# yg838457845/ORB_SLAM2-Chinese-annotation

Measured on AMD Instinct MI355X. Metric: frames/sec (extract+match) at 1241×376, 1000 feat/frame; 1/2/4/8 GPU, higher is better.
Workload: dtype u8; 1 GPU; C4: 1241x376 KITTI-shaped synthetic stream, 1000 feat/frame, SearchByProjection vs 5000-point local map per frame; distinct_frames_per_gpu=8192, frames_per_launch=1024, parallelism=single rank; no collective (one process, one GPU)

## Files before the change

orb_slam2-chinese-annotation_amd/csrc/extractor_kernels.hip:

```cpp
#include <stdlib.h>
#include <type_traits>
#include <algorithm>
#include "orb_device.h"
#include "orb_plan.h"
#include "orb_kernels.h"
#include "orb_pattern_data.h"
#include "../../include/orb_abi.h"

#define PYR_TW 128
#ifndef PYR_IMAGES_PER_WG
#define PYR_IMAGES_PER_WG 16
#endif
#define PYR_TH 32
#ifndef PYR_TARGET_WGS
#define PYR_TARGET_WGS 0
#endif
#define PYR_SROWS 44
#define PYR_SW 44
#define PYR_SROWS_WIDE 64
#define PYR_SW_WIDE 64

__global__ __launch_bounds__(256) void k_pyr_resize_generic(
    const uint8_t* __restrict__ src, long long srcImgPitch, int srcStride, int sw, int sh,
    uint8_t* __restrict__ dst, long long dstImgPitch, int dstStride, int dw, int dh,
// ... 1042 lines not shown
#if !FC_ROWMAJOR
      if (fresh)
        sc64[valid ? (o >> 3) : trashS] = last ? outsideLast : 0ull;
#endif
#if FC_ROWMAJOR
      const uint32_t X = __builtin_amdgcn_perm(rp[1], rp[0], 0x07050301u);
      const uint32_t Y = __builtin_amdgcn_perm(rp[3], rp[2], 0x07050301u);
      const uint32_t fails = ((X >> 7) & 0x01010101u) | ((Y >> 3) & 0x10101010u);
      uint32_t mk = ~((fails * 0x01020408u) >> 24) &
                    (valid ? (last ? (1u << nvLast) - 1u : 0xFFu) : 0u);
      const int cnt = __builtin_popcount(mk);
      int incl = wave_incl_scan(cnt);
      __asm__ volatile("" : "+v"(incl));
      int pos = nq + incl - cnt;
      while (mk) {
        const int j = __builtin_ctz(mk);
        mk &= mk - 1u;
        queue[pos++] = (uint16_t)(off + j);
      }
      nq += __builtin_amdgcn_readlane(incl, 63);
#else
      const unsigned long long vm = __ballot(valid), vIn = __ballot(valid && !last);
#pragma unroll
      for (int j = 0; j < 8; ++j) {
        const uint32_t w = rp[j >> 1];
        const bool sgn = (j & 1) ? ((int)w >= 0) : ((short)(w & 0xFFFFu) >= 0);
        const unsigned long long bj = __ballot(sgn) & (j < nvLast ? vm : vIn);
        const int pos = (int)__builtin_amdgcn_mbcnt_hi((uint32_t)(bj >> 32),
                                                       __builtin_amdgcn_mbcnt_lo((uint32_t)bj, (uint32_t)nq));
        queue[lane_select(bj, pos, trashQ)] = (uint16_t)(off + j);
        nq += __popcll(bj);
      }
#endif
      }
      k += kInc;
      off += dOff;
      if (k >= nK) {
        k -= nK;
        off += wrapOff;
      }
      if (nq > FC_QCAP - 512 || g0 + 64 >= nG) {
        wave_lds_sync();
        flush(t, fresh);
        wave_lds_sync();
      }
    }
  };
  auto nms = [&](int t) {
    for (int i = lane; i < 2 * ih; i += 64) bits[i] = 0;
    wave_lds_sync();
    const bool dense = nc > FC_CCAP;
    const int nItems = dense ? ih * iw : nc;
    for (int j = lane; j < nItems; j += 64) {
      int x, y, off;
      if (dense) {
        y = (int)(((float)j + 0.5f) * invW);
        x = j - y * iw;
        off = (y + 3) * P + (x + 8);
      } else {
        off = corners[j];
        const int ry = (int)(((float)off + 0.5f) * invP);
        y = ry - 3;
        x = off - ry * P - 8;
      }
      const uint8_t* cp = sc + off;
      const int m = cp[0];
      const int r0 = cp[-P - 1], r1 = cp[-P], r2 = cp[-P + 1], r3 = cp[-1], r4 = cp[1],
                r5 = cp[P - 1], r6 = cp[P], r7 = cp[P + 1];
      if (m <= t || m < 2) continue;
      const bool L = x > 0, Rt = x < iw - 1, U = y > 0, D = y < ih - 1;
      const int nb[8] = {(U && L) ? r0 : 0, U ? r1 : 0, (U && Rt) ? r2 : 0, L ? r3 : 0,
                         Rt ? r4 : 0, (D && L) ? r5 : 0, D ? r6 : 0, (D && Rt) ? r7 : 0};
      bool ok = true;
#pragma unroll
      for (int k = 0; k < 8; ++k) ok = ok && !(nb[k] > t && nb[k] >= m);
      if (ok) atomicOr(&bits[2 * y + (x >> 5)], 1u << (x & 31));
    }
    wave_lds_sync();
  };
  uint32_t* out = cellKeys + slot * plan.keyCap;
  auto nms_emit = [&](int t) -> int {
    const bool dense = nc > FC_CCAP;
    const int nItems = dense ? ih * iw : nc;
    const uint32_t kx0 = (uint32_t)(cd.x0 + 3), ky0 = (uint32_t)(cd.y0 + 3);
    int nOut = 0;
    for (int j0 = 0; j0 < nItems; j0 += 64) {
      const int j = j0 + lane;
      bool ok = false;
      int x = 0, y = 0, m = 0;
      if (j < nItems) {
        int off;
        if (dense) {
          y = (int)(((float)j + 0.5f) * invW);
          x = j - y * iw;
          off = (y + 3) * P + (x + 8);
        } else {
          off = corners[j];
          const int ry = (int)(((float)off + 0.5f) * invP);
          y = ry - 3;
          x = off - ry * P - 8;
        }
        int oq = off - P - 1;
        if (PT) __asm__ volatile("" : "+v"(oq));
        const uint8_t* cq = sc + oq;
        m = cq[P + 1];
        const int nb[8] = {cq[0], cq[1], cq[2], cq[P], cq[P + 2], cq[2 * P], cq[2 * P + 1],
                           cq[2 * P + 2]};
        ok = m > t && m >= 2;
#pragma unroll
        for (int k = 0; k < 8; ++k) ok = ok && !(nb[k] > t && nb[k] >= m);
      }
      const unsigned long long bal = __ballot(ok);
      const int pos = nOut + (int)__builtin_amdgcn_mbcnt_hi((uint32_t)(bal >> 32),
                                                            __builtin_amdgcn_mbcnt_lo((uint32_t)bal, 0u));
      if (ok) out[pos] = pack_key(kx0 + x, ky0 + y, m - 1);
      nOut += __popcll(bal);
    }
    return nOut;
  };
  auto compact = [&]() -> int {
    unsigned long long row = 0ull;
    if (lane < ih) {
      const uint2 w = *reinterpret_cast<const uint2*>(bits + 2 * lane);
      row = (unsigned long long)w.x | ((unsigned long long)w.y << 32);
    }
    const int cnt = __popcll(row);
    const int incl = wave_incl_scan(cnt);
    const int total = __builtin_amdgcn_readlane(incl, 63);
    int o = incl - cnt;
    const uint8_t* srow = sc + (lane + 3) * P + 8;
    const uint32_t kx = (uint32_t)(cd.x0 + 3), ky = (uint32_t)(cd.y0 + 3 + lane);
    while (row) {
      const int x0 = __builtin_ctzll(row);
      row &= row - 1;
      const bool two = row != 0;
      const int x1 = two ? __builtin_ctzll(row) : x0;
      if (two) row &= row - 1;
      const int m0 = srow[x0], m1 = srow[x1];
      out[o] = pack_key(kx + x0, ky, m0 - 1);
      if (two) out[o + 1] = pack_key(kx + x1, ky, m1 - 1);
      o += two ? 2 : 1;
    }
    return total;
  };
#if FC_ROWMAJOR
  (void)nms;
  (void)compact;
#endif
  fast_pass(ti, true);
#if FC_ROWMAJOR
  int n = nms_emit(ti);
#else
  nms(ti);
  int n = compact();
#endif
  if (n == 0 && tm != ti) {
    nc = 0;
    fast_pass(tm, false);
#if FC_ROWMAJOR
    n = nms_emit(tm);
#else
    nms(tm);
    n = compact();
#endif
  }
  if (lane == 0) cellCount[slot] = n;
  ci = ciNext;
  wave_lds_sync();
  }
}

struct OctNode {
  int16_t x0, y0, x1, y1;
  int cnt;
  int seq;
};

__device__ __forceinline__ int oct_quad(uint32_t key, const OctNode& n) {
  const int kx = key_x(key) - 16, ky = key_y(key) - 16;
  const int mx = n.x0 + ((n.x1 - n.x0 + 1) >> 1);
  const int my = n.y0 + ((n.y1 - n.y0 + 1) >> 1);
  return (kx < mx ? 0 : 1) + (ky < my ? 0 : 2);
}

__device__ __forceinline__ OctNode oct_child(const OctNode& p, int q, int cnt, int seq) {
  const int mx = p.x0 + ((p.x1 - p.x0 + 1) >> 1);
  const int my = p.y0 + ((p.y1 - p.y0 + 1) >> 1);
  OctNode c;
  c.x0 = (int16_t)((q & 1) ? mx : p.x0);
  c.x1 = (int16_t)((q & 1) ? p.x1 : mx);
  c.y0 = (int16_t)((q & 2) ? my : p.y0);
  c.y1 = (int16_t)((q & 2) ? p.y1 : my);
  c.cnt = cnt;
  c.seq = seq;
  return c;
}

__device__ int block_scan_array(int* a, int n, int* tmp) {
  const int T = blockDim.x, t = threadIdx.x;
  const int per = (n + T - 1) / T;
  const int b = min(t * per, n), e = min(b + per, n);
  int s = 0;
  for (int i = b; i < e; ++i) s += a[i];
  int total;
  int ex = block_excl_scan(s, tmp, &total);
  for (int i = b; i < e; ++i) {
    const int v = a[i];
    a[i] = ex;
    ex += v;
  }
  __syncthreads();
  return total;
}

__device__ void block_scan2(int* a, int na, int* b, int nb, int extra, int* tmp, int* totA,
                            int* totB, int* totX) {
  const int T = blockDim.x, t = threadIdx.x;
  const int pa = (na + T - 1) / T, pb = (nb + T - 1) / T;
  const int ba = min(t * pa, na), ea = min(ba + pa, na);
  const int bb = min(t * pb, nb), eb = min(bb + pb, nb);
  __syncthreads();
  int sa = 0, sb = 0;
  for (int i = ba; i < ea; ++i) sa += a[i];
  for (int i = bb; i < eb; ++i) sb += b[i];
  const int l = lane_id(), w = t >> 6, nw = (T + 63) >> 6;
  const int ia = wave_incl_scan(sa), ib = wave_incl_scan(sb), ix = wave_incl_scan(extra);
  if (l == 63) {
    tmp[w] = ia;
    tmp[16 + w] = ib;
    tmp[32 + w] = ix;
  }
  __syncthreads();
  if (t < 3) {
    int acc = 0;
    for (int i = 0; i < nw; ++i) {
      const int v = tmp[16 * t + i];
      tmp[16 * t + i] = acc;
      acc += v;
    }
    tmp[48 + t] = acc;
  }
  __syncthreads();
  int xa = tmp[w] + ia - sa, xb = tmp[16 + w] + ib - sb;
  *totA = tmp[48];
  *totB = tmp[49];
  *totX = tmp[50];
  for (int i = ba; i < ea; ++i) {
    const int v = a[i];
    a[i] = xa;
    xa += v;
  }
  for (int i = bb; i < eb; ++i) {
    const int v = b[i];
    b[i] = xb;
    xb += v;
  }
  __syncthreads();
}

__device__ void block_bitonic_desc(unsigned long long* v, int n2) {
  for (int k = 2; k <= n2; k <<= 1) {
    for (int j = k >> 1; j > 0; j >>= 1) {
      for (int i = threadIdx.x; i < n2; i += blockDim.x) {
        const int ixj = i ^ j;
        if (ixj > i) {
          const unsigned long long a = v[i], b = v[ixj];
          const bool descBlock = (i & k) == 0;
          if (descBlock ? (a < b) : (a > b)) {
            v[i] = b;
            v[ixj] = a;
          }
        }
      }
      __syncthreads();
    }
  }
}

#define OCT_RANK_MAX 512
template <int RQ>
__device__ __forceinline__ void oct_rank_by_count(unsigned long long* sortBuf, int ncand, int t, int T) {
  unsigned long long mine[RQ];
  int rank[RQ];
#pragma unroll
  for (int q = 0; q < RQ; ++q) {
    const int j = t + q * T;
    mine[q] = j < ncand ? sortBuf[j] : 0ull;
    rank[q] = 0;
  }
  for (int i = 0; i < ncand; ++i) {
    const unsigned long long k = sortBuf[i];
#pragma unroll
    for (int q = 0; q < RQ; ++q) rank[q] += k > mine[q];
  }
  __syncthreads();
#pragma unroll
  for (int q = 0; q < RQ; ++q)
    if (t + q * T < ncand) sortBuf[rank[q]] = mine[q];
  __syncthreads();
}

#define OCT_MAX_PASSES 512
#define OCT_REG_KEYS 8
#ifndef OCT_BATCH_THREADS
#define OCT_BATCH_THREADS 256
#endif
#ifndef OCT_REG_THREADS
#define OCT_REG_THREADS 512
#endif

template <bool REG, bool GNODES>
__global__ __launch_bounds__(512) void k_octree(
    OrbPlanDesc plan, const int32_t* __restrict__ cellCount, const uint32_t* __restrict__ cellKeys,
    uint32_t* __restrict__ gKeys, uint16_t* __restrict__ gNid, int ldsKeyCap, int nodeCapMax,
    int maxCellsPerLevel, uint32_t* __restrict__ outKeys, int32_t* __restrict__ outCount,
    int32_t* __restrict__ errFlag, int levelBeg, int maxPasses, unsigned char* __restrict__ gNodes,
    long long nodeStride) {
  extern __shared__ __attribute__((aligned(16))) unsigned char smem[];
  __shared__ int tmp[52];
  __shared__ int sh[8];
  const int l = levelBeg + blockIdx.y, img = blockIdx.x, T = blockDim.x, t = threadIdx.x;
  const OrbLevelDesc& L = plan.lv[l];
  const int NC = nodeCapMax;
  int n2 = 1;
  while (n2 < NC) n2 <<= 1;
  unsigned char* p = GNODES ? gNodes + ((long long)img * plan.nlevels + l) * nodeStride : smem;
  unsigned long long* sortBuf = (unsigned long long*)p; p += (size_t)n2 * 8;
  OctNode* A = (OctNode*)p; p += (size_t)NC * sizeof(OctNode);
  OctNode* B = (OctNode*)p; p += (size_t)NC * sizeof(OctNode);
  int* q4 = (int*)p; p += (size_t)NC * 16;
  int* g0 = (int*)p; p += (size_t)NC * 4;
  int* g1 = (int*)p; p += (size_t)NC * 4;
  int* g2 = (int*)p; p += (size_t)NC * 4;
  int* rk = (int*)p; p += (size_t)NC * 4;
  int* cellBase = (int*)p; p += (size_t)((maxCellsPerLevel + 3) & ~3) * 4;
  if (GNODES) p = smem;
  uint32_t* Klds = (uint32_t*)p; p += (size_t)ldsKeyCap * 4;
  uint16_t* Nlds = (uint16_t*)p;

  const int cb = L.cellBeg, nc = L.cellEnd - L.cellBeg;
  const long long cellSlot0 = (long long)img * plan.ncells + cb;
  for (int i = t; i < nc; i += T) cellBase[i] = cellCount[cellSlot0 + i];
  __syncthreads();
  const int n = block_scan_array(cellBase, nc, tmp);
  uint32_t* K;
  uint16_t* NID;
  if (n <= ldsKeyCap) {
    K = Klds;
    NID = Nlds;
  } else {
    K = gKeys + cellSlot0 * plan.keyCap;
    NID = gNid + cellSlot0 * plan.keyCap;
  }
  errFlag += img;
  for (int c = t; c < nc; c += T) {
    const int cnt = cellCount[cellSlot0 + c], base = cellBase[c];
    const uint32_t* src = cellKeys + (cellSlot0 + c) * plan.keyCap;
    for (int i = 0; i < cnt; ++i) K[base + i] = src[i];
  }
  const bool inReg = REG && n <= OCT_REG_KEYS * T;
  uint32_t kr[OCT_REG_KEYS];
  int nr[OCT_REG_KEYS];
  auto each_key = [&](auto&& f) {
    if (inReg) {
#pragma unroll
      for (int i = 0; i < OCT_REG_KEYS; ++i) {
        const int k = t + i * T;
        if (k < n) f(kr[i], nr[i], k);
      }
    } else {
      for (int k = t; k < n; k += T) {
        const uint32_t key = K[k];
        int nid = NID[k];
        f(key, nid, k);
        NID[k] = (uint16_t)nid;
      }
    }
  };
  __syncthreads();
  if (inReg) {
#pragma unroll
    for (int i = 0; i < OCT_REG_KEYS; ++i) {
      const int k = t + i * T;
      kr[i] = k < n ? K[k] : 0u;
      nr[i] = 0;
    }
  }
  const int nIni = L.nIni;
  const float hX = L.hX;
  for (int i = t; i < nIni; i += T) g0[i] = 0;
  __syncthreads();
  each_key([&](uint32_t key, int& nid, int) {
    const float xr = (float)(key_x(key) - 16);
    const int r = min((int)__fdiv_rn(xr, hX), nIni - 1);
    nid = r;
    atomicAdd(&g0[r], 1);
  });
  __syncthreads();
  if (t == 0) {
    int a = 0;
    for (int i = 0; i < nIni; ++i) {
      g1[i] = a;
      if (g0[i] > 0) {
        OctNode nd;
        nd.x0 = (int16_t)(int)(hX * (float)i);
        nd.x1 = (int16_t)(int)(hX * (float)(i + 1));
        nd.y0 = 0;
        nd.y1 = (int16_t)L.Hr;
        nd.cnt = g0[i];
        nd.seq = i;
        A[a++] = nd;
      }
    }
    sh[0] = a;
  }
  __syncthreads();
  each_key([&](uint32_t, int& nid, int) { nid = g1[nid]; });
  int alive = sh[0];
  const int N = L.quota;
  int seqNext = nIni;
  bool finalPhase = false;
  int pass = 0;
  __syncthreads();
  for (; pass < maxPasses; ++pass) {
    const int prev = alive;
    if (!finalPhase) {
      for (int i = t; i < alive * 4; i += T) q4[i] = 0;
      __syncthreads();
      each_key([&](uint32_t key, int& nid, int) {
        const OctNode nd = A[nid];
        if (nd.cnt > 1) atomicAdd(&q4[nid * 4 + oct_quad(key, nd)], 1);
      });
      __syncthreads();
      int nteLocal = 0;
      for (int a = t; a < alive; a += T) {
        int nce = 0;
        if (A[a].cnt > 1) {
#pragma unroll
          for (int q = 0; q < 4; ++q) {
            const int c = q4[a * 4 + q];
            nce += c > 0;
            nteLocal += c > 1;
          }
        }
        g0[a] = nce;
        g1[a] = A[a].cnt > 1 ? 0 : 1;
      }
      int nToExpand, S, NM;
      block_scan2(g0, alive, g1, alive, nteLocal, tmp, &S, &NM, &nToExpand);
      if (S + NM > NC) {
        if (t == 0) atomicOr(errFlag, 2);
        break;
      }
      for (int a = t; a < alive; a += T) {
        const OctNode nd = A[a];
        if (nd.cnt > 1) {
          int pos = g0[a];
#pragma unroll
          for (int q = 0; q < 4; ++q) {
            const int c = q4[a * 4 + q];
            if (c > 0) {
              const int ni = S - 1 - pos;
              B[ni] = oct_child(nd, q, c, seqNext + pos);
              q4[a * 4 + q] = ni;
              ++pos;
            }
          }
        } else {
          const int ni = S + g1[a];
          B[ni] = nd;
          q4[a * 4] = ni;
        }
      }
      __syncthreads();
      each_key([&](uint32_t key, int& nid, int) {
        const OctNode nd = A[nid];
        nid = q4[nid * 4 + (nd.cnt > 1 ? oct_quad(key, nd) : 0)];
      });
      __syncthreads();
      OctNode* sw = A; A = B; B = sw;
      alive = S + NM;
      seqNext += S;
      if (alive >= N || alive == prev) break;
      if (alive + nToExpand * 3 > N) finalPhase = true;
    } else {
      if (seqNext >= (1 << 24)) {
        if (t == 0) atomicOr(errFlag, 8);
        break;
      }
      for (int a = t; a < alive; a += T) g0[a] = A[a].cnt > 1 ? 1 : 0;
      __syncthreads();
      const int ncand = block_scan_array(g0, alive, tmp);
      if (ncand == 0) break;
      int m2 = 1;
      while (m2 < ncand) m2 <<= 1;
      for (int i = t; i < m2; i += T) sortBuf[i] = 0ull;
      __syncthreads();
      for (int a = t; a < alive; a += T) {
        const OctNode nd = A[a];
        if (nd.cnt > 1)
          sortBuf[g0[a]] = ((unsigned long long)nd.cnt << 40) |
                           ((unsigned long long)(uint32_t)nd.seq << 16) | (unsigned)a;
        q4[a * 4 + 0] = q4[a * 4 + 1] = q4[a * 4 + 2] = q4[a * 4 + 3] = 0;
        rk[a] = 0x7fffffff;
      }
      __syncthreads();
      if (ncand <= OCT_RANK_MAX) {
        if (T >= OCT_RANK_MAX)
          oct_rank_by_count<1>(sortBuf, ncand, t, T);
        else if (T >= 256)
          oct_rank_by_count<OCT_RANK_MAX / 256>(sortBuf, ncand, t, T);
        else
          oct_rank_by_count<OCT_RANK_MAX / 128>(sortBuf, ncand, t, T);
      } else {
        block_bitonic_desc(sortBuf, m2);
      }
      for (int j = t; j < ncand; j += T) rk[(int)(sortBuf[j] & 0xFFFF)] = j;
      each_key([&](uint32_t key, int& nid, int) {
        const OctNode nd = A[nid];
        if (nd.cnt > 1) atomicAdd(&q4[nid * 4 + oct_quad(key, nd)], 1);
      });
      if (t == 0) sh[1] = ncand - 1;
      __syncthreads();
      for (int j = t; j < ncand; j += T) {
        const int a = (int)(sortBuf[j] & 0xFFFF);
        int nce = 0;
#pragma unroll
        for (int q = 0; q < 4; ++q) nce += q4[a * 4 + q] > 0;
        g1[j] = nce;
        g2[j] = nce - 1;
      }
      __syncthreads();
      block_scan_array(g2, ncand, tmp);
      for (int j = t; j < ncand; j += T)
        if (alive + g2[j] + (g1[j] - 1) >= N) atomicMin(&sh[1], j);
      __syncthreads();
      const int jstop = sh[1];
      for (int j = t; j < ncand; j += T)
        if (j > jstop) g1[j] = 0;
      for (int a = t; a < alive; a += T) g2[a] = (rk[a] <= jstop) ? 0 : 1;
      int S, keep, unused;
      block_scan2(g1, ncand, g2, alive, 0, tmp, &S, &keep, &unused);
      if (S + keep > NC) {
        if (t == 0) atomicOr(errFlag, 2);
        break;
      }
      for (int a = t; a < alive; a += T) {
        const OctNode nd = A[a];
        const int j = rk[a];
        if (j <= jstop) {
          int pos = g1[j];
#pragma unroll
          for (int q = 0; q < 4; ++q) {
            const int c = q4[a * 4 + q];
            if (c > 0) {
              const int ni = S - 1 - pos;
              B[ni] = oct_child(nd, q, c, seqNext + pos);
              q4[a * 4 + q] = ni;
              ++pos;
            }
          }
        } else {
          const int ni = S + g2[a];
          B[ni] = nd;
          q4[a * 4] = ni;
        }
      }
      __syncthreads();
      each_key([&](uint32_t key, int& nid, int) {
        const OctNode nd = A[nid];
        nid = q4[nid * 4 + (rk[nid] <= jstop ? oct_quad(key, nd) : 0)];
      });
      __syncthreads();
      OctNode* sw = A; A = B; B = sw;
      alive = S + keep;
      seqNext += S;
      if (alive >= N || alive == prev) break;
    }
  }
  if (pass >= maxPasses && t == 0) atomicOr(errFlag, 4);
  uint32_t* best = (uint32_t*)g0;
  for (int a = t; a < alive; a += T) best[a] = 0u;
  __syncthreads();
  each_key([&](uint32_t key, int& nid, int k) {
    atomicMax(&best[nid], ((uint32_t)key_s(key) << 24) | (uint32_t)(0xFFFFFF - k));
  });
  __syncthreads();
  uint32_t* out = outKeys + (long long)img * plan.slotsPerImage + L.outOff;
  for (int a = t; a < alive; a += T) out[a] = K[0xFFFFFF - (int)(best[a] & 0xFFFFFF)];
  if (t == 0) outCount[img * plan.nlevels + l] = alive;
}

__constant__ int8_t c_pattern[2 * ORB_PATTERN_POINTS];
#define ORB_PATCH_DW 12
__constant__ int c_umax[16];
__constant__ uint32_t c_icmask[32][8];

__device__ __forceinline__ int reflect101(int i, int n) {
  if (n == 1) return 0;
  while (i < 0 || i >= n) {
    if (i < 0) i = -i;
    if (i >= n) i = 2 * n - 2 - i;
  }
  return i;
}

#define BLUR_SH (ORB_BLUR_TH + 6)
#define BLUR_WROW (ORB_BLUR_TW / 4 + 2)
#define BLUR_RP2 (ORB_BLUR_TW + 4)


__global__ __launch_bounds__(256) void k_blur_levels(
    const uint8_t* __restrict__ img0, long long img0Pitch, int img0Stride,
    const uint8_t* __restrict__ arena, long long arenaPitch, OrbPlanDesc plan,
    const OrbTileDesc* __restrict__ tiles, uint8_t* __restrict__ blur, long long blurPitch,
    int nImg) {
  __shared__ __attribute__((aligned(16))) uint32_t raw[BLUR_SH][BLUR_WROW + 1];
  __shared__ __attribute__((aligned(16))) uint32_t rowp2[BLUR_SH / 2][BLUR_RP2];
  const int tid = threadIdx.x;
  const OrbTileDesc td = tiles[blockIdx.x];
  const int l = td.level;
  const OrbLevelDesc& L = plan.lv[l];
  const int colA = td.x0 - 4;
  const bool rowsInside = td.y0 >= 3 && td.y0 + BLUR_SH - 3 <= L.h;
  auto level_of = [&](int im, int* pitch) -> const uint8_t* {
    if (l == 0) {
      *pitch = img0Stride;
      return img0 + (long long)im * img0Pitch;
    }
    *pitch = L.pitch;
    return arena + (long long)im * arenaPitch + L.arenaOff;
  };
  constexpr int NQ = (BLUR_SH * BLUR_WROW + 255) / 256;
  TilePrefetch<NQ> pf;
  const uint32_t magic = div_magic(BLUR_WROW);
  int pitch0;
  level_of(0, &pitch0);
  const bool alignedAll =
      l > 0 || ((img0Stride & 3) == 0 && (img0Pitch & 3) == 0 && (((uintptr_t)img0) & 3) == 0);
  const int cmax = alignedAll ? ((L.w - 1) & ~3) : L.w - 1;
  uint32_t eoff[NQ];
#pragma unroll
  for (int q = 0; q < NQ; ++q) {
    const uint32_t i = (uint32_t)min(q * 256 + tid, BLUR_SH * BLUR_WROW - 1);
    const int r = (int)__umulhi(i << 1, magic), c = (int)i - r * BLUR_WROW;
    const int y = td.y0 - 3 + r;
    eoff[q] = (uint32_t)((rowsInside ? y : reflect101(y, L.h)) * pitch0 + min(max(colA + 4 * c, 0), cmax));
  }
  auto issue = [&](int im) {
    int pitch;
    const uint8_t* lvl = level_of(im, &pitch);
    pf.issue(img_rsrc(lvl, (uint32_t)((L.h - 1) * pitch + L.w)), alignedAll, eoff);
  };
  int img = blockIdx.y;
  if (img >= nImg) return;
  issue(img);
  for (; img < nImg; img += gridDim.y) {
  pf.commit(&raw[0][0], BLUR_WROW + 1, BLUR_SH, BLUR_WROW, magic);
  if (img + (int)gridDim.y < nImg) issue(img + gridDim.y);
  const bool leftB = colA < 0, rightB = td.x0 + ORB_BLUR_TW + 3 > L.w;
  if (leftB || rightB) {
    __syncthreads();
    uint8_t* rb = reinterpret_cast<uint8_t*>(&raw[0][0]);
    constexpr int RB = (BLUR_WROW + 1) * 4;
    for (int i = tid; i < BLUR_SH * 7; i += 256) {
      const int r = i / 7, j = i - r * 7;
      const int x = j < 4 ? -4 + j : L.w + (j - 4);
      const int b = x - colA;
      if (b >= 0 && b < 4 * BLUR_WROW) {
        const int bs = reflect101(x, L.w) - colA;
        rb[r * RB + b] = (bs >= 0 && bs < 4 * BLUR_WROW) ? rb[r * RB + bs] : 0;
      }
    }
  }
  __syncthreads();
  constexpr uint32_t k0 = 18, k1 = 34, k2 = 49, k3 = 55, k4 = 49, k5 = 34, k6 = 18;
  constexpr uint32_t S0a = (k0 << 8) | (k1 << 16) | (k2 << 24), S0b = k3 | (k4 << 8) | (k5 << 16) | (k6 << 24);
  constexpr uint32_t S1a = (k0 << 16) | (k1 << 24), S1b = k2 | (k3 << 8) | (k4 << 16) | (k5 << 24), S1c = k6;
  constexpr uint32_t S2a = k0 << 24, S2b = k1 | (k2 << 8) | (k3 << 16) | (k4 << 24), S2c = k5 | (k6 << 8);
  constexpr uint32_t S3b = k0 | (k1 << 8) | (k2 << 16) | (k3 << 24), S3c = k4 | (k5 << 8) | (k6 << 16);
  constexpr int G = ORB_BLUR_TW / 4;
  for (int id = tid; id < (BLUR_SH / 2) * G; id += 256) {
    const int pr = id / G, g = id - pr * G;
    uint32_t o[2][4];
#pragma unroll
    for (int h = 0; h < 2; ++h) {
      const uint32_t* rw = raw[2 * pr + h] + g;
      const uint32_t w0 = rw[0], w1 = rw[1], w2 = rw[2];
      o[h][0] = __builtin_amdgcn_udot4(w0, S0a, __builtin_amdgcn_udot4(w1, S0b, 0u, false), false);
      o[h][1] = __builtin_amdgcn_udot4(w0, S1a, __builtin_amdgcn_udot4(w1, S1b,
                                       __builtin_amdgcn_udot4(w2, S1c, 0u, false), false), false);
      o[h][2] = __builtin_amdgcn_udot4(w0, S2a, __builtin_amdgcn_udot4(w1, S2b,
                                       __builtin_amdgcn_udot4(w2, S2c, 0u, false), false), false);
      o[h][3] = __builtin_amdgcn_udot4(w1, S3b, __builtin_amdgcn_udot4(w2, S3c, 0u, false), false);
    }
    uint4 pk;
    pk.x = o[0][0] | (o[1][0] << 16);
    pk.y = o[0][1] | (o[1][1] << 16);
    pk.z = o[0][2] | (o[1][2] << 16);
    pk.w = o[0][3] | (o[1][3] << 16);
    *reinterpret_cast<uint4*>(&rowp2[pr][4 * g]) = pk;
  }
  __syncthreads();
  typedef unsigned short u16x2 __attribute__((ext_vector_type(2)));
  const u16x2 E0 = {18, 34}, E1 = {49, 55}, E2 = {49, 34}, E3 = {18, 0};
  const u16x2 O0 = {0, 18}, O1 = {34, 49}, O2 = {55, 49}, O3 = {34, 18};
  const int qx = tid & (G - 1), qp = tid / G;
  uint8_t* dst = blur + (long long)img * blurPitch + L.blurOff;
  const int x = td.x0 + 4 * qx;
#pragma unroll
  for (int half = 0; half < 2; ++half) {
    const int pp = qp + 8 * half;
    uint4 pv[4];
#pragma unroll
    for (int k = 0; k < 4; ++k) pv[k] = *reinterpret_cast<const uint4*>(&rowp2[pp + k][4 * qx]);
    uint32_t packedE = 0, packedO = 0;
#pragma unroll
    for (int c = 0; c < 4; ++c) {
      uint32_t se = 0, so = 0;
#pragma unroll
      for (int k = 0; k < 4; ++k) {
        const uint32_t w = c == 0 ? pv[k].x : (c == 1 ? pv[k].y : (c == 2 ? pv[k].z : pv[k].w));
        const u16x2 v = __builtin_bit_cast(u16x2, w);
        se = __builtin_amdgcn_udot2(v, k == 0 ? E0 : (k == 1 ? E1 : (k == 2 ? E2 : E3)), se, false);
        so = __builtin_amdgcn_udot2(v, k == 0 ? O0 : (k == 1 ? O1 : (k == 2 ? O2 : O3)), so, false);
      }
      int ve = min((int)((se + (1u << 15)) >> 16), 255), vo = min((int)((so + (1u << 15)) >> 16), 255);
      __asm__ volatile("" : "+v"(ve), "+v"(vo));
      packedE |= (uint32_t)ve << (8 * c);
      packedO |= (uint32_t)vo << (8 * c);
    }
#pragma unroll
    for (int rr = 0; rr < 2; ++rr) {
      const int y = td.y0 + 2 * pp + rr;
      if (y >= L.h || x >= L.w) continue;
      const uint32_t packed = rr ? packedO : packedE;
      uint8_t* o = dst + (long long)y * L.blurPitch + x;
      if (x + 4 <= L.w) {
        *reinterpret_cast<uint32_t*>(o) = packed;
      } else {
        for (int c = 0; x + c < L.w; ++c) o[c] = (uint8_t)(packed >> (8 * c));
      }
    }
  }
  }
}

__device__ __forceinline__ int half_sum(int v) {
  v += __builtin_amdgcn_update_dpp(0, v, 0xB1, 0xF, 0xF, false);
  v += __builtin_amdgcn_update_dpp(0, v, 0x4E, 0xF, 0xF, false);
  v += __builtin_amdgcn_update_dpp(0, v, 0x141, 0xF, 0xF, false);
  v += __builtin_amdgcn_update_dpp(0, v, 0x140, 0xF, 0xF, false);
  v += __builtin_amdgcn_ds_swizzle(v, 0x401F);
  return v;
}

#ifndef DESC_RS_DW
#define DESC_RS_DW 40
#endif
#define DESC_RS_PAIRS 22
struct DescWaveLds {
  uint32_t rsp[2][DESC_RS_PAIRS][DESC_RS_DW];
};

#ifndef DESC_PPW
#define DESC_PPW 4
#endif
#ifndef DESC_MIN_WAVES
#define DESC_MIN_WAVES 0
#endif
#if DESC_MIN_WAVES > 0
#define DESC_LAUNCH_BOUNDS __launch_bounds__(256, DESC_MIN_WAVES)
#else
#define DESC_LAUNCH_BOUNDS __launch_bounds__(256)
#endif
#ifndef DESC_LDS_TABLES
#define DESC_LDS_TABLES 1
#endif
#ifndef DESC_MAGIC_ROUND
#define DESC_MAGIC_ROUND 1
#endif
#ifndef DESC_ROW37
#define DESC_ROW37 1
#endif
#ifndef DESC_SMALL_CT
#define DESC_SMALL_CT 1
#endif

template <int PPW>
__global__ DESC_LAUNCH_BOUNDS void k_orient_desc(
    const uint8_t* __restrict__ img0, long long img0Pitch, int img0Stride,
    const uint8_t* __restrict__ arena, long long arenaPitch, OrbPlanDesc plan,
    const uint32_t* __restrict__ outKeys, const int32_t* __restrict__ outCount,
    const int32_t* __restrict__ errFlag, orb_keypoint_t* __restrict__ kps,
    uint8_t* __restrict__ desc, int capacity, int32_t* __restrict__ counts, int ppwRt,
    int slotBeg, int slotEnd) {
  const int ppw = PPW ? PPW : ppwRt;
  __shared__ __attribute__((aligned(16))) DescWaveLds sm[4];
#if DESC_LDS_TABLES
  __shared__ __attribute__((aligned(16))) float4 sPat[ORB_PATTERN_POINTS / 2];
  __shared__ __attribute__((aligned(16))) uint4 sW[2];
  {
    const int t = threadIdx.x;
    sPat[t] = make_float4((float)c_pattern[4 * t], (float)c_pattern[4 * t + 1],
                          (float)c_pattern[4 * t + 2], (float)c_pattern[4 * t + 3]);
    if (t < 2)
      sW[t] = t == 0 ? make_uint4(18u | 34u << 16, 49u | 55u << 16, 49u | 34u << 16, 18u)
                     : make_uint4(18u << 16, 34u | 49u << 16, 55u | 49u << 16, 34u | 18u << 16);
    __syncthreads();
  }
#endif
  const int w = __builtin_amdgcn_readfirstlane(threadIdx.x >> 6), lane = threadIdx.x & 63;
  const int half = lane >> 5, hl = lane & 31;
  int bx, img;
  xcd_swizzle(bx, img);
  const int32_t* cnts = outCount + img * plan.nlevels;
  if (bx == 0 && threadIdx.x == 0 && slotEnd == plan.slotsPerImage) {
    int tot = 0;
    for (int i = 0; i < plan.nlevels; ++i) tot += cnts[i];
    counts[img] = errFlag[img] ? (int32_t)ORB_EDEVICE : tot;
  }
  const int pairBase = (slotBeg >> 1) + bx * 4 * ppw + w;
  if (2 * pairBase >= slotEnd) return;
  const uint32_t* imgKeys = outKeys + (long long)img * plan.slotsPerImage;
  uint32_t keyv = 0;
  if (lane < 2 * ppw) {
    const int slot = 2 * (pairBase + 4 * (lane >> 1)) + (lane & 1);
    if (slot < slotEnd) keyv = imgKeys[slot];
  }
  const int cntv = lane < plan.nlevels ? cnts[lane] : 0;
  const int cntx = wave_incl_scan(cntv) - cntv;
  const int offv = lane < plan.nlevels ? plan.lv[lane].outOff : INT_MAX;
  uint32_t (*rsp)[DESC_RS_DW] = sm[w].rsp[half];
  const bool second = hl < DESC_RS_PAIRS;
  struct Pair {
    bool valid, active;
    int l, i, cx, cy;
    uint32_t key, key0, key1;
  };
  auto setup = [&](int j) {
    Pair P;
    P.valid = false;
    const int slot0 = 2 * (pairBase + 4 * j);
    if (slot0 >= slotEnd) return P;
    const int l = __builtin_amdgcn_readfirstlane(__popcll(__ballot(offv <= slot0)) - 1);
    const int i0 = slot0 - __builtin_amdgcn_readlane(offv, l), nl = __builtin_amdgcn_readlane(cntv, l);
    if (i0 >= nl) return P;
    P.valid = true;
    P.l = l;
    P.active = i0 + half < nl;
    P.i = i0 + (P.active ? half : 0);
    const uint32_t k0 = __builtin_amdgcn_readlane(keyv, 2 * j);
    const uint32_t k1 = __builtin_amdgcn_readlane(keyv, 2 * j + 1);
    P.key = (half && P.active) ? k1 : k0;
    P.key0 = k0;
    P.key1 = i0 + 1 < nl ? k1 : k0;
    P.cx = key_x(P.key);
    P.cy = key_y(P.key);
    return P;
  };
  uint32_t ra[12], rb[12], sha = 0, shb = 0;
  auto issue = [&](const Pair& P) {
    const OrbLevelDesc& L = plan.lv[P.l];
    const uint8_t* lvl;
    int pitch;
    if (P.l == 0) {
      lvl = img0 + (long long)img * img0Pitch;
      pitch = img0Stride;
    } else {
      lvl = arena + (long long)img * arenaPitch + L.arenaOff;
      pitch = L.pitch;
    }
    const ImgRsrc im = img_rsrc(lvl, (uint32_t)((L.h - 1) * pitch + L.w));
    auto load_row = [&](int r, uint32_t* d) {
      int y = P.cy - 21 + r;
      y = y < 0 ? -y : (y >= L.h ? 2 * L.h - 2 - y : y);
      const int o = y * pitch + P.cx - 21 + (int)im.sh;
      const uint32_t a0 = o < 0 ? 0u : ((uint32_t)o & ~3u);
#pragma unroll
      for (int k = 0; k < 3; ++k) {
        const auto v = __builtin_amdgcn_raw_buffer_load_b128(im.r, (int)(a0 + 16 * k), 0, 0);
        d[4 * k] = (uint32_t)v[0];
        d[4 * k + 1] = (uint32_t)v[1];
        d[4 * k + 2] = (uint32_t)v[2];
        d[4 * k + 3] = (uint32_t)v[3];
      }
      return o < 0 ? 4u + (uint32_t)(-o) : ((uint32_t)o & 3u);
    };
    if (second) {
      sha = load_row(2 * hl, ra);
      shb = load_row(2 * hl + 1, rb);
    }
  };
// ... 528 lines not shown
```

Measured before the change: 354,900 frames/s.

## Fuse octree relabel with next-pass quadrant counting and add single-wave small-node path

Restructures the octree distribution kernel so that relabelling keys to child nodes and counting quadrants for the next pass happen in one sweep over keys, using double-buffered count tables swapped each pass. When 64 or fewer nodes are alive, the pass bookkeeping (scans, ranking, split selection) runs in a single wavefront with lane intrinsics instead of block-wide scans and barriers. Key gathering is rewritten as a per-key binary search over cell bases, and in-LDS key/node-id accesses are vectorised in groups of four through a templated LDS/global path. This cuts key sweeps and __syncthreads per pass, at the cost of more code, higher register pressure, and a more intricate correctness surface.

```diff
diff --git a/orb_slam2-chinese-annotation_amd/csrc/extractor_kernels.hip b/orb_slam2-chinese-annotation_amd/csrc/extractor_kernels.hip
--- a/orb_slam2-chinese-annotation_amd/csrc/extractor_kernels.hip
+++ b/orb_slam2-chinese-annotation_amd/csrc/extractor_kernels.hip
@@ -1368,6 +1368,10 @@
 
 #define OCT_MAX_PASSES 512
 #define OCT_REG_KEYS 8
+#define OCT_KB 4
+#ifndef OCT_GB
+#define OCT_GB 8
+#endif
 #ifndef OCT_BATCH_THREADS
 #define OCT_BATCH_THREADS 256
 #endif
@@ -1392,13 +1396,10 @@
   while (n2 < NC) n2 <<= 1;
   unsigned char* p = GNODES ? gNodes + ((long long)img * plan.nlevels + l) * nodeStride : smem;
   unsigned long long* sortBuf = (unsigned long long*)p; p += (size_t)n2 * 8;
-  OctNode* A = (OctNode*)p; p += (size_t)NC * sizeof(OctNode);
-  OctNode* B = (OctNode*)p; p += (size_t)NC * sizeof(OctNode);
-  int* q4 = (int*)p; p += (size_t)NC * 16;
-  int* g0 = (int*)p; p += (size_t)NC * 4;
-  int* g1 = (int*)p; p += (size_t)NC * 4;
-  int* g2 = (int*)p; p += (size_t)NC * 4;
-  int* rk = (int*)p; p += (size_t)NC * 4;
+  OctNode* nodeA = (OctNode*)p; p += (size_t)NC * sizeof(OctNode);
+  OctNode* nodeB = (OctNode*)p; p += (size_t)NC * sizeof(OctNode);
+  int* tabQ = (int*)p; p += (size_t)NC * 16;
+  int* tabG = (int*)p; p += (size_t)NC * 16;
   int* cellBase = (int*)p; p += (size_t)((maxCellsPerLevel + 3) & ~3) * 4;
   if (GNODES) p = smem;
   uint32_t* Klds = (uint32_t*)p; p += (size_t)ldsKeyCap * 4;
@@ -1409,39 +1410,120 @@
   for (int i = t; i < nc; i += T) cellBase[i] = cellCount[cellSlot0 + i];
   __syncthreads();
   const int n = block_scan_array(cellBase, nc, tmp);
-  uint32_t* K;
-  uint16_t* NID;
-  if (n <= ldsKeyCap) {
-    K = Klds;
-    NID = Nlds;
-  } else {
-    K = gKeys + cellSlot0 * plan.keyCap;
-    NID = gNid + cellSlot0 * plan.keyCap;
-  }
   errFlag += img;
-  for (int c = t; c < nc; c += T) {
-    const int cnt = cellCount[cellSlot0 + c], base = cellBase[c];
-    const uint32_t* src = cellKeys + (cellSlot0 + c) * plan.keyCap;
-    for (int i = 0; i < cnt; ++i) K[base + i] = src[i];
+  auto distribute = [&](uint32_t* __restrict__ K, uint16_t* __restrict__ NID,
+                        auto keysInLds) __attribute__((always_inline)) {
+  constexpr bool KLDS = decltype(keysInLds)::value;
+  static_assert(OCT_KB == 4 && OCT_REG_KEYS % OCT_KB == 0, "key blocks are four keys");
+  OctNode* A = nodeA;
+  OctNode* B = nodeB;
+  int* Q = tabQ;
+  int* G = tabG;
+  {
+    int ncp = 1;
+    while (ncp < nc) ncp <<= 1;
+    const int keyCap = plan.keyCap;
+    for (int k0 = t; k0 < n; k0 += OCT_GB * T) {
+      int kk[OCT_GB], c[OCT_GB];
+#pragma unroll
+      for (int u = 0; u < OCT_GB; ++u) {
+        kk[u] = min(k0 + u * T, n - 1);
+        c[u] = 0;
+      }
+      for (int s = ncp >> 1; s > 0; s >>= 1) {
+#pragma unroll
+        for (int u = 0; u < OCT_GB; ++u) {
+          const int m = c[u] + s;
+          if (cellBase[min(m, nc - 1)] <= kk[u] && m < nc) c[u] = m;
+        }
+      }
+      uint32_t v[OCT_GB];
+#pragma unroll
+      for (int u = 0; u < OCT_GB; ++u) {
+        const int i = min(kk[u] - cellBase[c[u]], keyCap - 1);
+        v[u] = cellKeys[(cellSlot0 + c[u]) * keyCap + i];
+      }
+#pragma unroll
+      for (int u = 0; u < OCT_GB; ++u)
+        if (k0 + u * T < n) K[k0 + u * T] = v[u];
+    }
   }
   const bool inReg = REG && n <= OCT_REG_KEYS * T;
   uint32_t kr[OCT_REG_KEYS];
   int nr[OCT_REG_KEYS];
-  auto each_key = [&](auto&& f) {
+  auto each_block = [&](bool loadN, bool storeN, auto&& f) __attribute__((always_inline)) {
     if (inReg) {
 #pragma unroll
-      for (int i = 0; i < OCT_REG_KEYS; ++i) {
-        const int k = t + i * T;
-        if (k < n) f(kr[i], nr[i], k);
+      for (int b = 0; b < OCT_REG_KEYS / OCT_KB; ++b) {
+        const int k0 = t + b * OCT_KB * T;
+        if (k0 < n) f(&kr[b * OCT_KB], &nr[b * OCT_KB], k0, T);
       }
     } else {
-      for (int k = t; k < n; k += T) {
-        const uint32_t key = K[k];
-        int nid = NID[k];
-        f(key, nid, k);
-        NID[k] = (uint16_t)nid;
-      }
-    }
+      for (int k0 = t * OCT_KB; k0 < n; k0 += T * OCT_KB) {
+        uint32_t key[OCT_KB];
+        int nid[OCT_KB];
+        if constexpr (KLDS) {
+          const uint4 kv = *(const uint4*)(K + k0);
+          key[0] = kv.x; key[1] = kv.y; key[2] = kv.z; key[3] = kv.w;
+          uint2 nv = make_uint2(0u, 0u);
+          if (loadN) nv = *(const uint2*)(NID + k0);
+          nid[0] = (int)(nv.x & 0xFFFFu); nid[1] = (int)(nv.x >> 16);
+          nid[2] = (int)(nv.y & 0xFFFFu); nid[3] = (int)(nv.y >> 16);
+#pragma unroll
+          for (int u = 0; u < OCT_KB; ++u)
+            if (k0 + u >= n) {
+              key[u] = 0u;
+              nid[u] = 0;
+            }
+        } else {
+#pragma unroll
+          for (int u = 0; u < OCT_KB; ++u) {
+            const bool ok = k0 + u < n;
+            key[u] = ok ? K[k0 + u] : 0u;
+            nid[u] = ok && loadN ? (int)NID[k0 + u] : 0;
+          }
+        }
+        f(key, nid, k0, 1);
+        if (storeN) {
+          if constexpr (KLDS) {
+            *(uint2*)(NID + k0) = make_uint2((uint32_t)nid[0] | ((uint32_t)nid[1] << 16),
+                                             (uint32_t)nid[2] | ((uint32_t)nid[3] << 16));
+          } else {
+#pragma unroll
+            for (int u = 0; u < OCT_KB; ++u)
+              if (k0 + u < n) NID[k0 + u] = (uint16_t)nid[u];
+          }
+        }
+      }
+    }
+  };
+  auto relabel_and_count = [&](bool cont) __attribute__((always_inline)) {
+    each_block(true, true, [&](const uint32_t* key, int* nid, int k0, int ks) __attribute__((always_inline)) {
+      OctNode nd[OCT_KB];
+      int ci[OCT_KB];
+#pragma unroll
+      for (int u = 0; u < OCT_KB; ++u) nd[u] = A[nid[u]];
+#pragma unroll
+      for (int u = 0; u < OCT_KB; ++u) {
+        const int v = Q[nid[u] * 4 + oct_quad(key[u], nd[u])];
+        ci[u] = k0 + u * ks < n ? v : 0;
+      }
+      if (cont) {
+        OctNode cn[OCT_KB];
+#pragma unroll
+        for (int u = 0; u < OCT_KB; ++u) cn[u] = B[ci[u]];
+#pragma unroll
+        for (int u = 0; u < OCT_KB; ++u)
+          if (k0 + u * ks < n) {
+            nid[u] = ci[u];
+            if (cn[u].cnt > 1) atomicAdd(&G[ci[u] * 4 + oct_quad(key[u], cn[u])], 1);
+          }
+      } else {
+#pragma unroll
+        for (int u = 0; u < OCT_KB; ++u)
+          if (k0 + u * ks < n) nid[u] = ci[u];
+      }
+    });
   };
   __syncthreads();
   if (inReg) {
@@ -1454,34 +1536,58 @@
   }
   const int nIni = L.nIni;
   const float hX = L.hX;
-  for (int i = t; i < nIni; i += T) g0[i] = 0;
-  __syncthreads();
-  each_key([&](uint32_t key, int& nid, int) {
-    const float xr = (float)(key_x(key) - 16);
-    const int r = min((int)__fdiv_rn(xr, hX), nIni - 1);
-    nid = r;
-    atomicAdd(&g0[r], 1);
-  });
-  __syncthreads();
-  if (t == 0) {
-    int a = 0;
-    for (int i = 0; i < nIni; ++i) {
-      g1[i] = a;
-      if (g0[i] > 0) {
-        OctNode nd;
-        nd.x0 = (int16_t)(int)(hX * (float)i);
-        nd.x1 = (int16_t)(int)(hX * (float)(i + 1));
-        nd.y0 = 0;
-        nd.y1 = (int16_t)L.Hr;
-        nd.cnt = g0[i];
-        nd.seq = i;
-        A[a++] = nd;
-      }
-    }
-    sh[0] = a;
-  }
-  __syncthreads();
-  each_key([&](uint32_t, int& nid, int) { nid = g1[nid]; });
+  {
+    int* const g0 = G;
+    int* const g1 = G + NC;
+    for (int i = t; i < nIni; i += T) {
+      g0[i] = 0;
+      *(int4*)&Q[i * 4] = make_int4(0, 0, 0, 0);
+    }
+    __syncthreads();
+    each_block(false, true, [&](const uint32_t* key, int* nid, int k0, int ks) __attribute__((always_inline)) {
+#pragma unroll
+      for (int u = 0; u < OCT_KB; ++u)
+        if (k0 + u * ks < n) {
+          const float xr = (float)(key_x(key[u]) - 16);
+          const int r = min((int)__fdiv_rn(xr, hX), nIni - 1);
+          nid[u] = r;
+          atomicAdd(&g0[r], 1);
+        }
+    });
+    __syncthreads();
+    if (t == 0) {
+      int a = 0;
+      for (int i = 0; i < nIni; ++i) {
+        g1[i] = a;
+        if (g0[i] > 0) {
+          OctNode nd;
+          nd.x0 = (int16_t)(int)(hX * (float)i);
+          nd.x1 = (int16_t)(int)(hX * (float)(i + 1));
+          nd.y0 = 0;
+          nd.y1 = (int16_t)L.Hr;
+          nd.cnt = g0[i];
+          nd.seq = i;
+          A[a++] = nd;
+        }
+      }
+      sh[0] = a;
+    }
+    __syncthreads();
+    each_block(true, true, [&](const uint32_t* key, int* nid, int k0, int ks) __attribute__((always_inline)) {
+      int v[OCT_KB];
+      OctNode nd[OCT_KB];
+#pragma unroll
+      for (int u = 0; u < OCT_KB; ++u) v[u] = k0 + u * ks < n ? g1[nid[u]] : 0;
+#pragma unroll
+      for (int u = 0; u < OCT_KB; ++u) nd[u] = A[v[u]];
+#pragma unroll
+      for (int u = 0; u < OCT_KB; ++u)
+        if (k0 + u * ks < n) {
+          nid[u] = v[u];
+          if (nd[u].cnt > 1) atomicAdd(&Q[v[u] * 4 + oct_quad(key[u], nd[u])], 1);
+        }
+    });
+  }
   int alive = sh[0];
   const int N = L.quota;
   int seqNext = nIni;
@@ -1490,21 +1596,112 @@
   __syncthreads();
   for (; pass < maxPasses; ++pass) {
     const int prev = alive;
-    if (!finalPhase) {
-      for (int i = t; i < alive * 4; i += T) q4[i] = 0;
+    int* const g0 = G;
+    int* const g1 = G + NC;
+    int* const g2 = G + 2 * NC;
+    int* const rk = G + 3 * NC;
+    int S, next;
+    const bool small = alive <= 64;
+    if (small) {
+      if (finalPhase && seqNext >= (1 << 24)) {
+        if (t == 0) atomicOr(errFlag, 8);
+        break;
+      }
+      if (t < 64) {
+        const int a = t;
+        const bool valid = a < alive;
+        const OctNode nd = A[valid ? a : 0];
+        const bool multi = valid && nd.cnt > 1;
+        const int4 cv = *(const int4*)&Q[(valid ? a : 0) * 4];
+        const int c[4] = {multi ? cv.x : 0, multi ? cv.y : 0, multi ? cv.z : 0, multi ? cv.w : 0};
+        int nce = 0, nte = 0;
+#pragma unroll
+        for (int q = 0; q < 4; ++q) {
+          nce += c[q] > 0;
+          nte += c[q] > 1;
+        }
+        bool divide, stop = false;
+        int pos, Sw, nExp = 0;
+        if (!finalPhase) {
+          divide = multi;
+          const int ia = wave_incl_scan(nce);
+          Sw = __builtin_amdgcn_readlane(ia, 63);
+          pos = ia - nce;
+          nExp = wave_sum(nte);
+        } else {
+          const int ncand = __popcll(__ballot(multi));
+          stop = ncand == 0;
+          const unsigned long long key =
+              multi ? ((unsigned long long)nd.cnt << 40) | ((unsigned long long)(uint32_t)nd.seq << 16) |
+                          (unsigned)a
+                    : 0ull;
+          const int klo = (int)(uint32_t)key, khi = (int)(uint32_t)(key >> 32);
+          int rank = 0;
+          for (int i = 0; i < 64; ++i) {
+            const unsigned long long ki =
+                ((unsigned long long)(uint32_t)__builtin_amdgcn_readlane(khi, i) << 32) |
+                (uint32_t)__builtin_amdgcn_readlane(klo, i);
+            rank += (ki > key || (ki == key && i < a)) ? 1 : 0;
+          }
+          const int nceS = __builtin_amdgcn_ds_permute(rank * 4, nce);
+          const bool candS = a < ncand;
+          const int d = candS ? nceS - 1 : 0;
+          const int g2x = wave_incl_scan(d) - d;
+          const unsigned long long hit = __ballot(candS && alive + g2x + nceS - 1 >= N);
+          const int jstop = hit ? __ffsll((long long)hit) - 1 : ncand - 1;
+          const int e = candS && a <= jstop ? nceS : 0;
+          const int ie = wave_incl_scan(e);
+          Sw = __builtin_amdgcn_readlane(ie, 63);
+          pos = __builtin_amdgcn_ds_bpermute(rank * 4, ie - e);
+          divide = multi && rank <= jstop;
+        }
+        const int keepf = valid && !divide ? 1 : 0;
+        const int ik = wave_incl_scan(keepf);
+        const int keepW = __builtin_amdgcn_readlane(ik, 63);
+        const int nextW = Sw + keepW;
+        if (!stop && nextW <= NC) {
+          const bool contW = nextW < N && nextW != prev && pass + 1 < maxPasses;
+          if (divide) {
+#pragma unroll
+            for (int q = 0; q < 4; ++q)
+              if (c[q] > 0) {
+                const int ni = Sw - 1 - pos;
+                B[ni] = oct_child(nd, q, c[q], seqNext + pos);
+                Q[a * 4 + q] = ni;
+                if (contW) *(int4*)&G[ni * 4] = make_int4(0, 0, 0, 0);
+                ++pos;
+              }
+          } else if (valid) {
+            const int ni = Sw + ik - keepf;
+            B[ni] = nd;
+            *(int4*)&Q[a * 4] = make_int4(ni, ni, ni, ni);
+            if (contW) *(int4*)&G[ni * 4] = make_int4(0, 0, 0, 0);
+          }
+        }
+        if (t == 0) {
+          sh[2] = Sw;
+          sh[3] = nextW;
+          sh[4] = nExp;
+          sh[5] = stop ? 1 : 0;
+        }
+      }
       __syncthreads();
-      each_key([&](uint32_t key, int& nid, int) {
-        const OctNode nd = A[nid];
-        if (nd.cnt > 1) atomicAdd(&q4[nid * 4 + oct_quad(key, nd)], 1);
-      });
-      __syncthreads();
+      if (sh[5]) break;
+      S = sh[2];
+      next = sh[3];
+      if (next > NC) {
+        if (t == 0) atomicOr(errFlag, 2);
+        break;
+      }
+      if (!finalPhase && next + sh[4] * 3 > N) finalPhase = true;
+    } else if (!finalPhase) {
       int nteLocal = 0;
       for (int a = t; a < alive; a += T) {
         int nce = 0;
         if (A[a].cnt > 1) {
 #pragma unroll
           for (int q = 0; q < 4; ++q) {
-            const int c = q4[a * 4 + q];
+            const int c = Q[a * 4 + q];
             nce += c > 0;
             nteLocal += c > 1;
           }
@@ -1512,7 +1709,7 @@
         g0[a] = nce;
         g1[a] = A[a].cnt > 1 ? 0 : 1;
       }
-      int nToExpand, S, NM;
+      int nToExpand, NM;
       block_scan2(g0, alive, g1, alive, nteLocal, tmp, &S, &NM, &nToExpand);
       if (S + NM > NC) {
         if (t == 0) atomicOr(errFlag, 2);
@@ -1524,31 +1721,22 @@
           int pos = g0[a];
 #pragma unroll
           for (int q = 0; q < 4; ++q) {
-            const int c = q4[a * 4 + q];
+            const int c = Q[a * 4 + q];
             if (c > 0) {
               const int ni = S - 1 - pos;
               B[ni] = oct_child(nd, q, c, seqNext + pos);
-              q4[a * 4 + q] = ni;
+              Q[a * 4 + q] = ni;
               ++pos;
             }
           }
         } else {
           const int ni = S + g1[a];
           B[ni] = nd;
-          q4[a * 4] = ni;
+          *(int4*)&Q[a * 4] = make_int4(ni, ni, ni, ni);
         }
       }
-      __syncthreads();
-      each_key([&](uint32_t key, int& nid, int) {
-        const OctNode nd = A[nid];
-        nid = q4[nid * 4 + (nd.cnt > 1 ? oct_quad(key, nd) : 0)];
-      });
-      __syncthreads();
-      OctNode* sw = A; A = B; B = sw;
-      alive = S + NM;
-      seqNext += S;
-      if (alive >= N || alive == prev) break;
-      if (alive + nToExpand * 3 > N) finalPhase = true;
+      next = S + NM;
+      if (next + nToExpand * 3 > N) finalPhase = true;
     } else {
       if (seqNext >= (1 << 24)) {
         if (t == 0) atomicOr(errFlag, 8);
@@ -1567,7 +1755,6 @@
         if (nd.cnt > 1)
           sortBuf[g0[a]] = ((unsigned long long)nd.cnt << 40) |
                            ((unsigned long long)(uint32_t)nd.seq << 16) | (unsigned)a;
-        q4[a * 4 + 0] = q4[a * 4 + 1] = q4[a * 4 + 2] = q4[a * 4 + 3] = 0;
         rk[a] = 0x7fffffff;
       }
       __syncthreads();
@@ -1582,17 +1769,13 @@
         block_bitonic_desc(sortBuf, m2);
       }
       for (int j = t; j < ncand; j += T) rk[(int)(sortBuf[j] & 0xFFFF)] = j;
-      each_key([&](uint32_t key, int& nid, int) {
-        const OctNode nd = A[nid];
-        if (nd.cnt > 1) atomicAdd(&q4[nid * 4 + oct_quad(key, nd)], 1);
-      });
       if (t == 0) sh[1] = ncand - 1;
       __syncthreads();
       for (int j = t; j < ncand; j += T) {
         const int a = (int)(sortBuf[j] & 0xFFFF);
         int nce = 0;
 #pragma unroll
-        for (int q = 0; q < 4; ++q) nce += q4[a * 4 + q] > 0;
+        for (int q = 0; q < 4; ++q) nce += Q[a * 4 + q] > 0;
         g1[j] = nce;
         g2[j] = nce - 1;
       }
@@ -1605,7 +1788,7 @@
       for (int j = t; j < ncand; j += T)
         if (j > jstop) g1[j] = 0;
       for (int a = t; a < alive; a += T) g2[a] = (rk[a] <= jstop) ? 0 : 1;
-      int S, keep, unused;
+      int keep, unused;
       block_scan2(g1, ncand, g2, alive, 0, tmp, &S, &keep, &unused);
       if (S + keep > NC) {
         if (t == 0) atomicOr(errFlag, 2);
@@ -1618,43 +1801,59 @@
           int pos = g1[j];
 #pragma unroll
           for (int q = 0; q < 4; ++q) {
-            const int c = q4[a * 4 + q];
+            const int c = Q[a * 4 + q];
             if (c > 0) {
               const int ni = S - 1 - pos;
               B[ni] = oct_child(nd, q, c, seqNext + pos);
-              q4[a * 4 + q] = ni;
+              Q[a * 4 + q] = ni;
               ++pos;
             }
           }
         } else {
           const int ni = S + g2[a];
           B[ni] = nd;
-          q4[a * 4] = ni;
+          *(int4*)&Q[a * 4] = make_int4(ni, ni, ni, ni);
         }
       }
+      next = S + keep;
+    }
+    const bool cont = next < N && next != prev && pass + 1 < maxPasses;
+    if (!small) {
       __syncthreads();
-      each_key([&](uint32_t key, int& nid, int) {
-        const OctNode nd = A[nid];
-        nid = q4[nid * 4 + (rk[nid] <= jstop ? oct_quad(key, nd) : 0)];
-      });
-      __syncthreads();
-      OctNode* sw = A; A = B; B = sw;
-      alive = S + keep;
-      seqNext += S;
-      if (alive >= N || alive == prev) break;
-    }
+      if (cont) {
+        for (int i = t; i < next; i += T) *(int4*)&G[i * 4] = make_int4(0, 0, 0, 0);
+        __syncthreads();
+      }
+    }
+    relabel_and_count(cont);
+    __syncthreads();
+    OctNode* sw = A; A = B; B = sw;
+    int* st = Q; Q = G; G = st;
+    alive = next;
+    seqNext += S;
+    if (alive >= N || alive == prev) break;
   }
   if (pass >= maxPasses && t == 0) atomicOr(errFlag, 4);
-  uint32_t* best = (uint32_t*)g0;
+  uint32_t* best = (uint32_t*)G;
   for (int a = t; a < alive; a += T) best[a] = 0u;
   __syncthreads();
-  each_key([&](uint32_t key, int& nid, int k) {
-    atomicMax(&best[nid], ((uint32_t)key_s(key) << 24) | (uint32_t)(0xFFFFFF - k));
+  each_block(true, false, [&](const uint32_t* key, int* nid, int k0, int ks) __attribute__((always_inline)) {
+#pragma unroll
+    for (int u = 0; u < OCT_KB; ++u) {
+      const int k = k0 + u * ks;
+      if (k < n)
+        atomicMax(&best[nid[u]], ((uint32_t)key_s(key[u]) << 24) | (uint32_t)(0xFFFFFF - k));
+    }
   });
   __syncthreads();
   uint32_t* out = outKeys + (long long)img * plan.slotsPerImage + L.outOff;
   for (int a = t; a < alive; a += T) out[a] = K[0xFFFFFF - (int)(best[a] & 0xFFFFFF)];
   if (t == 0) outCount[img * plan.nlevels + l] = alive;
+  };
+  if (n <= ldsKeyCap)
+    distribute(Klds, Nlds, std::true_type{});
+  else
+    distribute(gKeys + cellSlot0 * plan.keyCap, gNid + cellSlot0 * plan.keyCap, std::false_type{});
 }
 
 __constant__ int8_t c_pattern[2 * ORB_PATTERN_POINTS];
```

Measured after the change: 359,100 frames/s (median of 6 runs). 1.2% higher.
